# HighCWu/ControlLoRA

Measured on AMD Instinct MI355X. Metric: train images/sec SD-1.5+ControlLoRA 512^2 bs4/GPU, higher is better.
Workload: dtype f16; 1 GPU; configs/fill50k.json on SD-1.5 topology (seeded random weights), 512x512, bs=4/GPU, fp16; hot path = hint encoder + UNet fwd/bwd + adapter AdamW; latents/text embeddings synthetic (VAE/CLIP outside the hot path); global_batch=4, parallelism=dp1, hipgraph=True, allreduce_bytes=24188160, rccl_ranks=1, comm=torch, comm_requested=auto

## Files before the change

### controllora_amd/capi.py

```python
from __future__ import annotations

import ctypes as C
import os
from typing import Optional

import torch

_HERE = os.path.dirname(os.path.abspath(__file__))
LIB_PATH = os.environ.get("CLORA_LIB_PATH") or os.path.join(_HERE, "_build", "libclora.so")

ABI_VERSION = 4
OK, ERR_ARG, ERR_LAUNCH, ERR_WORKSPACE = 0, -1, -2, -3
_ERR = {ERR_ARG: "bad argument", ERR_LAUNCH: "kernel launch failed", ERR_WORKSPACE: "workspace too small"}


class CloraError(RuntimeError):
    pass


class ConvDesc(C.Structure):
    _fields_ = [(n, C.c_int) for n in (
        "enabled", "Hin", "Win", "Cin", "Hout", "Wout", "ksize", "mul", "kmul", "off", "lim_h", "lim_w", "shift",
        "need_even", "kchunk")]

# ... 90 lines not shown
    _fields_ = [("A", C.c_void_p), ("lda", C.c_int), ("T", C.c_void_p), ("ldt", C.c_int), ("toff", C.c_int), ("G", C.c_void_p),
                ("gs_n", C.c_int), ("gs_j", C.c_int), ("M", C.c_int), ("N", C.c_int), ("R", C.c_int), ("scale", C.c_float),
                ("a_rows", C.c_int), ("A2", C.c_void_p), ("lda2", C.c_int)]


class ConvPackJob(C.Structure):
    _fields_ = [("w", C.c_void_p), ("fwd", C.c_void_p), ("dgrad", C.c_void_p), ("Co", C.c_int), ("Ci", C.c_int), ("ksize", C.c_int),
                ("Cip", C.c_int), ("Cop", C.c_int), ("pad_", C.c_int)]


class ConvUnpackJob(C.Structure):
    _fields_ = [("stage", C.c_void_p), ("stage_b", C.c_void_p), ("grad_w", C.c_void_p), ("grad_b", C.c_void_p), ("Co", C.c_int),
                ("Ci", C.c_int), ("ksize", C.c_int), ("Cip", C.c_int)]


class SamplerCoef(C.Structure):
    _fields_ = [(n, C.c_float) for n in ("guidance", "x0_x", "x0_e", "k_x", "k_x0", "k_h", "k_e", "k_n")]


class ConvActJob(C.Structure):
    _fields_ = [("x", C.c_void_p), ("ldx", C.c_int), ("w", C.c_void_p), ("bias", C.c_void_p), ("y", C.c_void_p), ("ldy", C.c_int),
                ("Cin", C.c_int), ("Cout", C.c_int), ("relu", C.c_int)]


CONV_ACT_MAX_JOBS = 2
LORA_MAX_JOBS = 16
LORA_WGRAD_MAX_JOBS = 32
WGRAD_JOBS_PER_LAUNCH = min(LORA_WGRAD_MAX_JOBS, max(1, int(os.environ.get("CLORA_WGRAD_JOBS", "32"))))
CONV_MAX_JOBS = 32
CANNY_MAX_GROUP = 64
_P, _I, _Z, _F, _LL = C.c_void_p, C.c_int, C.c_size_t, C.c_float, C.c_longlong
_PROTOS = {
    "clora_gemm_f16": [_P, _I, _P, _P, _I, _I, _I, _I, C.POINTER(ConvDesc), C.POINTER(Epilogue), _I, _P, _Z, _P],
    "clora_gemm_f16_ex": [_P, _I, _P, _P, _I, _I, _I, _I, C.POINTER(ConvDesc), C.POINTER(Epilogue), _I, _I, _P, _Z, _P],
    "clora_conv_patch_eligible": [_I, C.POINTER(ConvDesc), _I],
    "clora_conv_strip_eligible": [_I, _I, C.POINTER(ConvDesc)],
    "clora_set_option": [C.c_char_p, _I],
    "clora_conv_wgrad_f16": [_P, _I, _P, _I, _P, _P, _I, _I, _I, C.POINTER(ConvDesc), _I, _P],
    "clora_conv_weight_pack_f32": [_P, _I, _I, _I, _I, _I, _P, _P, _P],
    "clora_conv_wgrad_unpack_f32": [_P, _P, _P, _P, _I, _I, _I, _I, _P],
    "clora_conv_weight_pack_multi_f32": [C.POINTER(ConvPackJob), _I, _P],
    "clora_conv_wgrad_unpack_multi_f32": [C.POINTER(ConvUnpackJob), _I, _P],
    "clora_attn_fwd_f16": [_P, _I, _P, _I, _P, _I, _P, _I, _P, _I, _I, _I, _I, _I, _F, _P],
    "clora_attn_max_head_dim": [_I],
    "clora_attn_fwd_causal_f16": [_P, _I, _P, _I, _P, _I, _P, _I, _I, _I, _I, _I, _F, _P],
    "clora_attn_bwd_f16": [_P, _I, _P, _I, _P, _I, _P, _I, _P, _I, _P, _P, _P, _I, _P, _I, _P, _I, _I, _I, _I, _I, _I, _F, _P, _Z, _P],
    "clora_groupnorm_fwd_f16": [_P, _P, _P, _P, _P, _I, _I, _I, _I, _F, _I, _P, _Z, _P],
    "clora_groupnorm_bwd_f16": [_P, _P, _P, _P, _P, _P, _P, _P, _P, _I, _I, _I, _I, _I, _I, _P, _Z, _P],
    "clora_groupnorm_fwd_f16_ex": [_P, _P, _I, C.POINTER(Deferred), _P, _P, _P, _P, _P, _I, _I, _I, _I, _F, _I, _P, _Z, _P],
    "clora_groupnorm_bwd_f16_ex": [_P, _P, C.POINTER(Deferred), _P, _P, _P, _I, _P, _P, _P, _P, _P, _I, _I, _I, _I, _I, _I, _P, _Z, _P],
    "clora_groupnorm_fwd_f16_team": [_P, _P, _I, C.POINTER(Deferred), _P, _P, _P, _P, _P, _I, _I, _I, _I, _F, _I, _P, _Z, _P, _Z, _P],
    "clora_groupnorm_fwd_f16_lo": [_P, _P, _I, C.POINTER(Deferred), _P, _P, _P, _P, _P, _I, _I, _I, _I, _F, _I, _P, _Z, _P, _Z, _P, _P, _P],
    "clora_layernorm_fwd_f16_lo": [_P, _P, _P, _P, _I, _I, _F, _P, _P],
    "clora_groupnorm_bwd_f16_team": [_P, _P, C.POINTER(Deferred), _P, _P, _P, _I, _P, _P, _P, _P, _P, _I, _I, _I, _I, _I, _I, _P, _Z, _P, _Z, _P],
    "clora_layernorm_bwd_f16_ex": [_P, _P, C.POINTER(Deferred), _P, _P, _P, _I, _I, _F, _P],
    "clora_finish_deferred": [C.POINTER(Deferred), _P],
    "clora_gemm_ln_fusable": [_I, _I, _I, _I, _I],
    "clora_gemm_tile_info": [_I, C.POINTER(GemmTile)],
    "clora_gemm_tile_at": [_I, C.POINTER(GemmTile)],
    "clora_gemm_fused_down_tile": [_I, _I, _I, C.POINTER(_I)],
    "clora_layernorm_fwd_f16": [_P, _P, _P, _P, _I, _I, _F, _P],
    "clora_softmax_rows_f16": [_P, _P, _I, _I, _I, _F, _P],
    "clora_layernorm_bwd_f16": [_P, _P, _P, _P, _P, _I, _I, _F, _P],
    "clora_geglu_fwd_f16": [_P, _P, _I, _I, _P],
    "clora_geglu_bwd_f16": [_P, _P, _P, _I, _I, _P],
    "clora_lora_down_f16": [_P, _I, _P, _I, _P, _I, _I, _I, _I, _I, _I, _I, _I, _F, _P],
    "clora_lora_down_multi_f16": [C.POINTER(LoraDownJob), _I, _P],
    "clora_lora_wgrad_multi_f16": [C.POINTER(LoraWgradJob), _I, _P, _Z, _P],
    "clora_lora_pack_f16": [_P, _I, _I, _P],
# ... 58 lines not shown
        self.cdll = C.CDLL(path)
        got = self.cdll.clora_abi_version() if hasattr(self.cdll, "clora_abi_version") else -1
        if got != ABI_VERSION and os.environ.get("CLORA_ABI_ANY", "") != "1":
            raise CloraError(f"{path} reports ABI {got}, this binding is written for ABI {ABI_VERSION} (include/clora.h); rebuild with "
                             "`python -m controllora_amd.build` (CLORA_ABI_ANY=1 overrides for A/B runs of older builds whose "
                             "struct layouts are known to match)")
        for name, argtypes in _PROTOS.items():
            if not hasattr(self.cdll, name) and os.environ.get("CLORA_ABI_ANY", "") == "1":
                continue
            fn = getattr(self.cdll, name)
            fn.argtypes = argtypes
            fn.restype = C.c_int
        self.cdll.clora_build_info.restype = C.c_char_p
        self.cdll.clora_groupnorm_workspace_bytes.restype = C.c_size_t
        self.cdll.clora_groupnorm_team_state_bytes.restype = C.c_size_t
        self.cdll.clora_lora_wgrad_workspace_bytes.restype = C.c_size_t
        self.cdll.clora_rank_gram_ws_bytes.restype = C.c_size_t
        if hasattr(self.cdll, "clora_conv_act_workspace"):
            self.cdll.clora_conv_act_workspace.restype = C.c_size_t
        self._options_from_env()
        self._derived = {}

    def derived(self, key, make):
        if key not in self._derived:
            self._derived[key] = make(self)
        return self._derived[key]

    def tiles(self) -> dict:
        def read(L):
            rows, r = {}, GemmTile()
# ... 58 lines not shown
```

### controllora_amd/csrc/clora_norm.hip

```cpp
#include <stdlib.h>
#include "clora_common.h"
#include "../../include/clora.h"
#include "clora_epilogue.h"

namespace {

constexpr int kMaxCols = 2;
constexpr int kLnCols = 4;

struct GnArgs {
    const half_t* x;
    const half_t* dy;
    const half_t* dres;
    half_t* y;
    const float* gamma;
    const float* beta;
    float* stats;
    float* partial;
    float* chpart;
    float* dgamma;
    float* dbeta;
    int B, HW, C, G, nchunk, rows_per_chunk;
    int accumulate_params;
    int params_in_apply;
// ... 464 lines not shown
                }
                if (r < r_end && cc < CH) {
                    const GnColW dc = gn_dx_col(p, cb + cc * 8);
                    st8(dc.p + ((size_t)b * p.HW + r) * dc.pitch, o);
                }
            }
        }
    }
}

__global__ __launch_bounds__(256) void gn_bwd_params_kernel(GnArgs p) {
    __shared__ float red[256 * 2];
    gn_bwd_params_block(p, blockIdx.x, red);
}

template <int NT>
__device__ __forceinline__ void gn_res_reduce(float* red, float* chs, const float (&a)[8], const float (&b)[8], int t, int CS, int cpg, int gps,
                                              int rl, int nrl, int c0, bool active, const float* weight, float* out2, float inv_n) {
    const int W = CS * 2;
    if (active) {
#pragma unroll
        for (int e = 0; e < 8; ++e) { red[rl * W + (c0 * 8 + e) * 2] = a[e]; red[rl * W + (c0 * 8 + e) * 2 + 1] = b[e]; }
    }
    __syncthreads();
    int seg = 1;
    while (seg < 8 && seg * 2 * CS <= NT) seg *= 2;
    {
        const int c = t / seg, sg = t - c * seg;
        float sa = 0.f, sb = 0.f;
        if (c < CS)
// ... 87 lines not shown
    gn_unpack8(ba, bb, bet);
    gn_affine8(mr, c0 * 8, cpg, gam, bet, sc, sh);
    half_t* ybase = p.y + (size_t)b * p.HW * p.C + cb + c0 * 8;
#pragma unroll
    for (int k = 0; k < NPT; ++k) {
        const int r = rl + k * nrl;
        half8 o;
        GN_NORM8(LO, v[k], w[k], lcol.m, sc, sh, p.fuse_silu, o)
        if (k < npt && r < p.HW) {
            st8(ybase + (size_t)r * p.C, o);
            if (p.xcopy) st8(p.xcopy + (size_t)b * p.HW * p.C + cb + c0 * 8 + (size_t)r * p.C, v[k]);
        }
    }
}

template <int NT, int NPT, bool DEF = false>
__global__ __launch_bounds__(NT) void gn_bwd_resident_kernel(GnArgs p) {
    __shared__ float red[NT * 16];
    __shared__ float chs[256 * 8 * 2];
    __shared__ float gs[64 * 2];
    const int t = threadIdx.x, b = blockIdx.z, cb = blockIdx.y * p.CS;
    const int CH = p.CS / 8, cpg = p.C / p.G, gps = p.G / p.nslab;
    const int nrl = NT / CH, rl = t / CH, c0 = t - rl * CH;
    const bool active = rl < nrl;
    const int npt = (p.HW + nrl - 1) / nrl;
    const size_t boff = (size_t)b * p.HW * p.C + cb + c0 * 8;
    float mean[8], rstd[8], sc[8], sh[8];
#pragma unroll
    for (int e = 0; e < 8; ++e) {
        const int ch = cb + (active ? c0 : 0) * 8 + e;
        const float* st = p.stats + ((size_t)b * p.G + ch / cpg) * 2;
// ... 21 lines not shown
#pragma unroll
        for (int k = 0; k < NPT; ++k) {
            const bool ok = k < npt && rl + k * nrl < p.HW;
#pragma unroll
            for (int e = 0; e < 8; ++e) {
                const float xf = (float)xv[k][e];
                const float xh = (xf - mean[e]) * rstd[e];
                float d = ok ? (float)gv[k][e] : 0.f;
                if (p.fuse_silu) d *= dsilu_f(xf * sc[e] + sh[e]);
                a1[e] += d;
                a2[e] += d * xh;
            }
        }
    }
    gn_res_reduce<NT>(red, chs, a1, a2, t, p.CS, cpg, gps, rl, nrl, c0, active, p.gamma + cb, gs, 1.0f / ((float)p.HW * (float)cpg));
    if (!active) return;
    float k2[8], k3[8];
#pragma unroll
    for (int e = 0; e < 8; ++e) {
        const int g = (c0 * 8 + e) / cpg;
        k2[e] = -rstd[e] * rstd[e] * gs[g * 2 + 1];
        k3[e] = -k2[e] * mean[e] - rstd[e] * gs[g * 2];
    }
    const bool has_res = p.dres != nullptr;
    const GnColW dxc = gn_dx_col(p, cb + c0 * 8);
#pragma unroll
    for (int k = 0; k < NPT; ++k) {
        const int r = rl + k * nrl;
        if (!(k < npt && r < p.HW)) continue;
        const size_t off = boff + (size_t)r * p.C;
// ... 119 lines not shown
    gn_unpack8(ba, bb, bet);
    gn_affine8(mr, c0 * 8, cpg, gam, bet, sc, sh);
    half_t* ybase = p.y + (size_t)b * p.HW * p.C + cb + c0 * 8;
#pragma unroll
    for (int k = 0; k < NPT; ++k) {
        const int r = r0 + rl + k * nrl;
        half8 o;
        GN_NORM8(LO, v[k], w[k], lcol.m, sc, sh, p.fuse_silu, o)
        if (r < r_end) {
            st8(ybase + (size_t)r * p.C, o);
            if (p.xcopy) st8(p.xcopy + (size_t)b * p.HW * p.C + cb + c0 * 8 + (size_t)r * p.C, v[k]);
        }
    }
}

template <int NT, int NPT>
__global__ __launch_bounds__(NT) void gn_bwd_team_kernel(GnArgs p) {
    __shared__ float red[NT * 16];
    __shared__ float chs[NT * 2];
    __shared__ float gs[64 * 2];
    __shared__ float gat[NT];
    __shared__ unsigned s_epoch;
    const int t = threadIdx.x;
    const int U = p.B * p.nslab, u = blockIdx.x % U, m = blockIdx.x / U;
    const int b = u / p.nslab, cb = (u - b * p.nslab) * p.CS;
    if (t == 0) s_epoch = CLORA_LD_AGENT_U32(p.tm_gen + u) + 1u;
    const int CH = p.CS / 8, cpg = p.C / p.G, gps = p.G / p.nslab;
    const int nrl = NT / CH, rl = t / CH, c0 = t - rl * CH;
    const bool active = rl < nrl;
    const int r0 = m * p.tm_rpb;
    const int r_end = (r0 + p.tm_rpb < p.HW) ? r0 + p.tm_rpb : p.HW;
// ... 22 lines not shown
#pragma unroll
        for (int k = 0; k < NPT; ++k) {
            const bool ok = r0 + rl + k * nrl < r_end;
#pragma unroll
            for (int e = 0; e < 8; ++e) {
                const float xf = (float)xv[k][e];
                const float xh = (xf - mean[e]) * rstd[e];
                float d = ok ? (float)gv[k][e] : 0.f;
                if (p.fuse_silu) d *= dsilu_f(xf * sc[e] + sh[e]);
                a1[e] += d;
                a2[e] += d * xh;
            }
        }
    }
    gn_res_reduce<NT>(red, chs, a1, a2, t, p.CS, cpg, gps, rl, nrl, c0, active, p.gamma + cb, gs, 1.0f);
    if (!gn_team_exchange<NT>(p, u, m, s_epoch, gps * 2, gs, gat, 1.0f / ((float)p.HW * (float)cpg))) return;
    if (!active) return;
    float k2[8], k3[8];
#pragma unroll
    for (int e = 0; e < 8; ++e) {
        const int g = (c0 * 8 + e) / cpg;
        k2[e] = -rstd[e] * rstd[e] * gs[g * 2 + 1];
        k3[e] = -k2[e] * mean[e] - rstd[e] * gs[g * 2];
    }
    const bool has_res = p.dres != nullptr;
    const GnColW dxc = gn_dx_col(p, cb + c0 * 8);
#pragma unroll
    for (int k = 0; k < NPT; ++k) {
        const int r = r0 + rl + k * nrl;
        if (!(r < r_end)) continue;
// ... 330 lines not shown
    }
}
size_t gn_workspace_bytes(const GnArgs& a, bool params) {
    size_t need = (size_t)a.B * a.nchunk * a.G * 2;
    if (params) need += (size_t)a.B * a.nchunk * a.C * 2;
    return need * sizeof(float);
}
int gn_bind_workspace(GnArgs& a, void* ws, size_t ws_bytes, bool params) {
    if (!ws || ws_bytes < gn_workspace_bytes(a, params)) return CLORA_ERR_WORKSPACE;
    a.partial = (float*)ws;
    a.chpart = params ? a.partial + (size_t)a.B * a.nchunk * a.G * 2 : nullptr;
    return CLORA_OK;
}

struct GnResident { int nt, npt; };
GnResident gn_resident_plan(GnArgs& a, bool bwd, bool params) {
    GnResident none = {0, 0};
    if (!clora_option(CLORA_OPT_GN_RESIDENT) || params) return none;
    const int cpg = a.C / a.G;
    int unit = 1;
    while ((unit * cpg) & 7) ++unit;
    if (a.G % unit) return none;
    int groups = unit;
    while (groups * cpg < 40 && groups * 2 <= a.G && a.G % (groups * 2) == 0) groups *= 2;
    const int CS = groups * cpg, CH = CS / 8;
    if (groups > 64 || CH > 256) return none;
    const int max_npt = bwd ? 8 : 16;
    for (int nt = 256; nt <= 512; nt *= 2) {
        const int nrl = nt / CH, npt = (a.HW + nrl - 1) / nrl;
        if (npt <= max_npt && groups * 8 <= nt && CS <= nt) {
            a.nslab = a.G / groups; a.CS = CS; a.nchunk = 1; a.rows_per_chunk = a.HW;
            GnResident r = {nt, npt <= 4 ? 4 : (npt <= 8 ? 8 : 16)};
            return r;
        }
    }
    return none;
}

int gn_team_plan(GnArgs& a, bool bwd, bool params, void* state, size_t state_bytes) {
    const int level = clora_option(CLORA_OPT_GN_TEAM);
    const int min_hw = level >= 4 ? 64 : ((level == 3 || (bwd && level == 2)) ? 256 : 1024);
    if (!state || state_bytes < kTeamStateBytes || params || !level || a.HW < min_hw) return 0;
    static int cus = -1;
    if (cus < 0) {
        int dev = 0, n = 0;
        if (hipGetDevice(&dev) != hipSuccess || hipDeviceGetAttribute(&n, hipDeviceAttributeMultiprocessorCount, dev) != hipSuccess) n = 0;
        cus = n;
    }
    if (cus < kTeamBlocks) return 0;
    const int cpg = a.C / a.G;
    int unit = 1;
    while ((unit * cpg) & 7) ++unit;
    if (a.G % unit) return 0;
    const int nunits = a.G / unit;
    int pick = 0, pick_npt = 0;
    for (int d = 1; d <= nunits; ++d) {
        if (nunits % d) continue;
        const int U = a.B * d;
        if (U > kTeamUnits || (kTeamBlocks % U)) continue;
        const int NB = kTeamBlocks / U, CS = a.C / d, CH = CS / 8, gps = a.G / d, GK = 2 * gps;
        if (NB < 2 || CS > kTeamNT || GK > kTeamGran || gps * 8 > kTeamNT) continue;
        if (NB > 8 * (kTeamNT / GK)) continue;
        const int nrl = kTeamNT / CH, rpb = clora_cdiv(a.HW, NB), npt = clora_cdiv(rpb, nrl);
        if (npt > (bwd ? 8 : 16)) continue;
        if (!pick || CS >= 160) { pick = d; pick_npt = npt; }
        if (CS < 160) break;
    }
    if (!pick) return 0;
    a.nslab = pick; a.CS = a.C / pick; a.nchunk = 1; a.rows_per_chunk = a.HW;
    a.tm_nb = kTeamBlocks / (a.B * pick); a.tm_rpb = clora_cdiv(a.HW, a.tm_nb);
    a.tm_err = (unsigned*)state; a.tm_gen = (unsigned*)((char*)state + 256);
    a.tm_gran = (unsigned long long*)((char*)state + kTeamHeader);
    a.tm_spin = 1u << 16; a.tm_probe = 0;
    return pick_npt <= 4 ? 4 : (pick_npt <= 8 ? 8 : 16);
}

enum GnForm { kGnTwoLaunch, kGnResident, kGnTeam };
struct GnLaunchPlan {
    GnForm form;
    int nt, npt;
    int nj, uf;
    bool deferred_here;
};
GnLaunchPlan gn_launch_plan(GnArgs& a, bool bwd, bool params, bool deferred, void* team_state, size_t team_state_bytes) {
    GnLaunchPlan pl = {kGnTwoLaunch, 0, 0, 1, 1, false};
    const GnResident res = gn_resident_plan(a, bwd, params);
    const bool fold_shape = res.nt && res.npt <= clora_option(CLORA_OPT_DEFER_MAX_ROWS);
    pl.deferred_here = deferred && fold_shape;
    if (!fold_shape && (!res.nt || clora_option(CLORA_OPT_GN_TEAM) >= 2)) {
        GnArgs ta = a;
        const int npt = gn_team_plan(ta, bwd, params, team_state, team_state_bytes);
        if (npt) {
            a = ta;
            pl.form = kGnTeam; pl.nt = kTeamNT; pl.npt = npt;
            return pl;
        }
    }
    if (res.nt) {
        pl.form = kGnResident; pl.nt = res.nt; pl.npt = res.npt;
        return pl;
    }
    gn_plan(a);
    pl.nj = a.CS / 8 > 256 ? 2 : 1;
    pl.uf = (pl.nj == 1 && clora_option(CLORA_OPT_GN_UNROLL)) ? 2 : 1;
    return pl;
}

template <bool BWD, bool DEF, bool LO>
void gn_resident_launch(const GnArgs& a, int nt, int npt, hipStream_t s) {
    static_assert(!(BWD && LO) && !(DEF && LO), "no such instantiation");
    const dim3 grid(1, a.nslab, a.B);
    if constexpr (BWD) {
        if (nt == 256 && npt == 4) hipLaunchKernelGGL((gn_bwd_resident_kernel<256, 4, DEF>), grid, dim3(256), 0, s, a);
        else if (nt == 256) hipLaunchKernelGGL((gn_bwd_resident_kernel<256, 8, DEF>), grid, dim3(256), 0, s, a);
        else hipLaunchKernelGGL((gn_bwd_resident_kernel<512, 8, DEF>), grid, dim3(512), 0, s, a);
    } else {
        if (nt == 256 && npt == 4) hipLaunchKernelGGL((gn_fwd_resident_kernel<256, 4, DEF, LO>), grid, dim3(256), 0, s, a);
        else if (nt == 256 && npt == 8) hipLaunchKernelGGL((gn_fwd_resident_kernel<256, 8, DEF, LO>), grid, dim3(256), 0, s, a);
        else if (nt == 256) hipLaunchKernelGGL((gn_fwd_resident_kernel<256, 16, DEF, LO>), grid, dim3(256), 0, s, a);
        else if (npt <= 8) hipLaunchKernelGGL((gn_fwd_resident_kernel<512, 8, DEF, LO>), grid, dim3(512), 0, s, a);
        else hipLaunchKernelGGL((gn_fwd_resident_kernel<512, 16, DEF, LO>), grid, dim3(512), 0, s, a);
    }
}

template <bool BWD, bool LO, int NJ, int UF>
void gn_two_launch_as(GnArgs& a, hipStream_t s) {
    const dim3 grid(a.nchunk, a.nslab, a.B), block(256);
    if constexpr (BWD) {
        static_assert(!LO, "no such instantiation");
        hipLaunchKernelGGL((gn_bwd_partial_kernel<NJ, UF>), grid, block, 0, s, a);
        a.params_in_apply = (a.dgamma && (long)a.nchunk * a.nslab * a.B >= clora_cdiv(a.C, 32)) ? 1 : 0;
        if (a.dgamma && !a.params_in_apply) hipLaunchKernelGGL(gn_bwd_params_kernel, dim3(clora_cdiv(a.C, 32)), block, 0, s, a);
        hipLaunchKernelGGL((gn_bwd_apply2_kernel<NJ, UF>), grid, block, 0, s, a);
    } else {
        hipLaunchKernelGGL((gn_fwd_partial_kernel<NJ, UF, LO>), grid, block, 0, s, a);
        hipLaunchKernelGGL((gn_fwd_apply2_kernel<NJ, UF, LO>), grid, block, 0, s, a);
    }
}
template <bool BWD, bool LO>
void gn_two_launch(GnArgs& a, int nj, int uf, hipStream_t s) {
    if (nj == 2) gn_two_launch_as<BWD, LO, 2, 1>(a, s);
    else if (uf == 2) gn_two_launch_as<BWD, LO, 1, 2>(a, s);
    else gn_two_launch_as<BWD, LO, 1, 1>(a, s);
}

template <bool BWD, bool LO = false>
void gn_team_launch(GnArgs& a, int npt, hipStream_t s) {
    const dim3 grid(kTeamBlocks), block(kTeamNT);
    for (int pass = CLORA_SEQUENTIAL_BLOCKS ? 0 : 1; pass < 2; ++pass) {
        a.tm_probe = pass == 0;
        if (BWD) {
            if (npt == 4) hipLaunchKernelGGL((gn_bwd_team_kernel<kTeamNT, 4>), grid, block, 0, s, a);
            else hipLaunchKernelGGL((gn_bwd_team_kernel<kTeamNT, 8>), grid, block, 0, s, a);
        } else {
            if (npt == 4) hipLaunchKernelGGL((gn_fwd_team_kernel<kTeamNT, 4, LO>), grid, block, 0, s, a);
            else if (npt == 8) hipLaunchKernelGGL((gn_fwd_team_kernel<kTeamNT, 8, LO>), grid, block, 0, s, a);
            else hipLaunchKernelGGL((gn_fwd_team_kernel<kTeamNT, 16, LO>), grid, block, 0, s, a);
        }
    }
}

int ew_blocks(size_t n) {
    size_t b = (n + 255) / 256;
    return (int)(b > 4096 ? 4096 : (b < 1 ? 1 : b));
}

}

// ... 22 lines not shown
    const bool lo = x_lo || x2_lo;
    if (lo && src && src->splits > 0) return CLORA_ERR_ARG;
    if (!gn_shape_ok(B, HW, C, G)) return CLORA_ERR_ARG;
    hipStream_t s = (hipStream_t)stream;
    const bool deferred = src && src->splits > 0;
    if (deferred) {
        if (x2 || !deferred_fits(src, B * HW, C)) return CLORA_ERR_ARG;
        x = src->C;
    }
    if (!x || (x2 && (Ca <= 0 || Ca >= C || (Ca & 7)))) return CLORA_ERR_ARG;
    GnArgs a = GnArgs();
    a.x = (const half_t*)x; a.y = (half_t*)y; a.gamma = gamma; a.beta = beta; a.stats = stats;
    a.B = B; a.HW = HW; a.C = C; a.G = G; a.eps = eps; a.fuse_silu = fuse_silu;
    a.x2 = (const half_t*)x2; a.Ca = x2 ? Ca : C; a.xcopy = (half_t*)xcopy;
    a.x_lo = (const half_t*)x_lo; a.x2_lo = (const half_t*)x2_lo;
    const GnLaunchPlan pl = gn_launch_plan(a, false, false, deferred, team_state, team_state_bytes);
    if (deferred && !pl.deferred_here) {
        const int rc = clora_finish_deferred(src, stream);
        if (rc != CLORA_OK) return rc;
    }
    if (pl.form == kGnTeam) {
        if (lo) gn_team_launch<false, true>(a, pl.npt, s);
        else gn_team_launch<false>(a, pl.npt, s);
    } else if (pl.form == kGnResident) {
        if (pl.deferred_here) {
            a.fin_partial = src->partial; a.fin_splits = src->splits; a.fin_epi = src->epi; a.xcopy = (half_t*)src->C;
            gn_resident_launch<false, true, false>(a, pl.nt, pl.npt, s);
        } else if (lo) {
            gn_resident_launch<false, false, true>(a, pl.nt, pl.npt, s);
        } else {
            gn_resident_launch<false, false, false>(a, pl.nt, pl.npt, s);
// ... 31 lines not shown
    return gn_fwd_impl(x, x2, Ca, src, xcopy, y, gamma, beta, stats, B, HW, C, G, eps, fuse_silu, team_state, team_state_bytes, workspace,
                       workspace_bytes, stream, x_lo, x2_lo);
}

extern "C" int clora_groupnorm_fwd_f16(const clora_half* x, clora_half* y, const float* gamma, const float* beta,
                                       float* stats, int B, int HW, int C, int G, float eps, int fuse_silu,
                                       void* workspace, size_t workspace_bytes, void* stream) {
    return clora_groupnorm_fwd_f16_ex(x, nullptr, 0, nullptr, nullptr, y, gamma, beta, stats, B, HW, C, G, eps, fuse_silu, workspace,
                                      workspace_bytes, stream);
}

namespace {
int gn_bwd_impl(const clora_half* x, const clora_half* dy, const clora_deferred_t* dy_src, const clora_half* dres,
                clora_half* dx, clora_half* dx2, int Ca, const float* gamma, const float* beta,
                const float* stats, float* dgamma, float* dbeta, int B, int HW, int C, int G, int fuse_silu,
                int accumulate_params, void* team_state, size_t team_state_bytes, void* workspace, size_t workspace_bytes, void* stream) {
    if (!x || !dx || !gamma || !beta || !stats || ((dgamma == nullptr) != (dbeta == nullptr))) return CLORA_ERR_ARG;
    if (!gn_shape_ok(B, HW, C, G)) return CLORA_ERR_ARG;
    if (dx2 && (Ca <= 0 || Ca >= C || (Ca & 7))) return CLORA_ERR_ARG;
    const bool deferred = dy_src && dy_src->splits > 0;
    if (deferred) {
        if (!deferred_fits(dy_src, B * HW, C)) return CLORA_ERR_ARG;
        dy = dy_src->C;
    }
    if (!dy) return CLORA_ERR_ARG;
    GnArgs a = GnArgs();
    a.x = (const half_t*)x; a.dy = (const half_t*)dy; a.dres = (const half_t*)dres; a.y = (half_t*)dx; a.gamma = gamma; a.beta = beta;
    a.stats = const_cast<float*>(stats); a.dgamma = dgamma; a.dbeta = dbeta;
    a.B = B; a.HW = HW; a.C = C; a.G = G; a.fuse_silu = fuse_silu; a.accumulate_params = accumulate_params;
    a.y2 = (half_t*)dx2; a.Ca = dx2 ? Ca : C;
    hipStream_t s = (hipStream_t)stream;
    const bool params = dgamma != nullptr;
    const GnLaunchPlan pl = gn_launch_plan(a, true, params, deferred, team_state, team_state_bytes);
    if (deferred && !pl.deferred_here) {
        const int rc = clora_finish_deferred(dy_src, stream);
        if (rc != CLORA_OK) return rc;
    }
    if (pl.form == kGnTeam) {
        gn_team_launch<true>(a, pl.npt, s);
    } else if (pl.form == kGnResident) {
        if (pl.deferred_here) {
            a.fin_partial = dy_src->partial; a.fin_splits = dy_src->splits; a.fin_epi = dy_src->epi;
            gn_resident_launch<true, true, false>(a, pl.nt, pl.npt, s);
        } else {
            gn_resident_launch<true, false, false>(a, pl.nt, pl.npt, s);
        }
    } else {
        const int rc = gn_bind_workspace(a, workspace, workspace_bytes, params);
        if (rc != CLORA_OK) return rc;
        gn_two_launch<true, false>(a, pl.nj, pl.uf, s);
    }
    return clora_check_launch();
}
}

extern "C" int clora_groupnorm_bwd_f16_ex(const clora_half* x, const clora_half* dy, const clora_deferred_t* dy_src, const clora_half* dres,
                                          clora_half* dx, clora_half* dx2, int Ca, const float* gamma, const float* beta,
                                          const float* stats, float* dgamma, float* dbeta, int B, int HW, int C, int G, int fuse_silu,
                                          int accumulate_params, void* workspace, size_t workspace_bytes, void* stream) {
    return gn_bwd_impl(x, dy, dy_src, dres, dx, dx2, Ca, gamma, beta, stats, dgamma, dbeta, B, HW, C, G, fuse_silu, accumulate_params, nullptr, 0,
                       workspace, workspace_bytes, stream);
}

extern "C" int clora_groupnorm_bwd_f16_team(const clora_half* x, const clora_half* dy, const clora_deferred_t* dy_src, const clora_half* dres,
                                            clora_half* dx, clora_half* dx2, int Ca, const float* gamma, const float* beta,
                                            const float* stats, float* dgamma, float* dbeta, int B, int HW, int C, int G, int fuse_silu,
                                            int accumulate_params, void* team_state, size_t team_state_bytes, void* workspace,
                                            size_t workspace_bytes, void* stream) {
    return gn_bwd_impl(x, dy, dy_src, dres, dx, dx2, Ca, gamma, beta, stats, dgamma, dbeta, B, HW, C, G, fuse_silu, accumulate_params, team_state,
                       team_state_bytes, workspace, workspace_bytes, stream);
}

extern "C" int clora_groupnorm_bwd_f16(const clora_half* x, const clora_half* dy, const clora_half* dres, clora_half* dx, const float* gamma,
                                       const float* beta, const float* stats, float* dgamma, float* dbeta, int B,
                                       int HW, int C, int G, int fuse_silu, int accumulate_params, void* workspace,
                                       size_t workspace_bytes, void* stream) {
    return clora_groupnorm_bwd_f16_ex(x, dy, nullptr, dres, dx, nullptr, 0, gamma, beta, stats, dgamma, dbeta, B, HW, C, G, fuse_silu,
                                      accumulate_params, workspace, workspace_bytes, stream);
}

namespace {
int ln_fwd_impl(const clora_half* x, clora_half* y, const float* gamma, const float* beta, int M, int C, float eps,
                const clora_half* x_lo, void* stream) {
    if (!x || !y || !gamma || !beta || M <= 0 || C <= 0 || (C & 7) || C / 8 > 64 * kLnCols) return CLORA_ERR_ARG;
    LnArgs a = LnArgs();
// ... 55 lines not shown
```

### controllora_amd/kernels.py

```python
from __future__ import annotations

import ctypes as C
import os
from typing import Optional, Tuple

import torch

from . import capi
from .capi import ConvDesc, Epilogue, ptr

f16, f32 = torch.float16, torch.float32


class KernelProfiler:

    def __init__(self, detail=False):
        self.detail = detail
        self.records = []

    def summary(self):
        torch.cuda.synchronize()
        agg = {}
        for name, e0, e1, fl, by in self.records:
            a = agg.setdefault(name, dict(calls=0, ms=0.0, flops=0.0, bytes=0.0))
# ... 482 lines not shown
    if split_at:
        dx = torch.empty((B, HW, split_at), dtype=f16, device=x.device)
        dx2 = torch.empty((B, HW, Cc - split_at), dtype=f16, device=x.device)
    else:
        dx, dx2 = torch.empty_like(x), None
    dg = db = None
    if grads_into is not None:
        dg, db = grads_into
        want_param_grads = True
    elif want_param_grads:
        dg = torch.empty(Cc, dtype=f32, device=x.device)
        db = torch.empty(Cc, dtype=f32, device=x.device)
    ws = _gn_ws(B, HW, Cc, G, x.device, True, want_param_grads)
    assert dres is None or (dres.shape == x.shape and dres.is_contiguous())
    team = gn_team_state(x.device)
    _call("clora_groupnorm_bwd_f16_team", ptr(x, f16), ptr(dy, f16), C.byref(dy_src) if dy_src is not None else None,
          ptr(dres, f16) if dres is not None else None, ptr(dx), ptr(dx2) if dx2 is not None else None, int(split_at),
          ptr(gamma, f32), ptr(beta, f32), ptr(stats, f32),
          ptr(dg, f32) if dg is not None else None, ptr(db, f32) if db is not None else None, B, HW, Cc, G, int(silu),
          int(grads_into is not None), ptr(team), team.numel(), ptr(ws), ws.numel())
    if split_at:
        dx = (dx, dx2)
    return (dx, None, None) if grads_into is not None else (dx, dg, db)


def layernorm_fwd(x, gamma, beta, eps, x_lo=None):
    x2 = _c2(x)
    y = torch.empty_like(x)
    if x_lo is not None:
        assert x_lo.shape == x.shape and x_lo.is_contiguous()
        _call("clora_layernorm_fwd_f16_lo", ptr(x2, f16), ptr(y), ptr(gamma, f32), ptr(beta, f32), x2.shape[0], x2.shape[1], float(eps),
              ptr(x_lo, f16))
        return y
    _call("clora_layernorm_fwd_f16", ptr(x2, f16), ptr(y), ptr(gamma, f32), ptr(beta, f32), x2.shape[0], x2.shape[1], float(eps))
    return y


def layernorm_bwd(x, dy, gamma, eps, dres=None):
# ... 183 lines not shown


def lora_wgrad_multi(jobs, device):
    groups = {}
    for j in jobs:
        groups.setdefault(4 if j.R <= 4 else (8 if j.R <= 8 else 16), []).append(j)
    wsb = capi.lib().cdll.clora_lora_wgrad_workspace_bytes
    for _, js in groups.items():
        for i in range(0, len(js), capi.WGRAD_JOBS_PER_LAUNCH):
            chunk = js[i:i + capi.WGRAD_JOBS_PER_LAUNCH]
            ws = workspace(sum(wsb(j.M, j.N, j.R) for j in chunk), device)
            arr = (capi.LoraWgradJob * len(chunk))(*chunk)
            _call("clora_lora_wgrad_multi_f16", arr, len(chunk), ptr(ws), ws.numel(), nbytes=sum(2.0 * j.M * j.N for j in chunk))


_wgrad_queue = {"jobs": [], "refs": [], "task": None, "enabled": os.environ.get("CLORA_DEFER_WGRAD", "1") != "0", "unpack": []}
DEFER_UNPACK = os.environ.get("CLORA_DEFER_UNPACK", "1") != "0"


def _graph_task_id():
    f = getattr(torch._C, "_current_graph_task_id", None)
    return f() if f is not None else -1


def _defer_open():
    if not _wgrad_queue["enabled"] or PROFILER is not None:
        return False
    task = _graph_task_id()
    if task < 0:
        return False
    if _wgrad_queue["task"] != task:
        lora_wgrad_discard()
# ... 10 lines not shown
    _wgrad_queue["refs"].extend(keepalive)
    _wgrad_queue["device"] = device


def conv_unpack_defer(job, *keepalive) -> bool:
    if not DEFER_UNPACK or not _defer_open():
        return False
    _wgrad_queue["unpack"].append(job)
    _wgrad_queue["refs"].extend(keepalive)
    return True


def lora_wgrad_discard():
    _wgrad_queue["jobs"].clear()
    _wgrad_queue["unpack"].clear()
    _wgrad_queue["refs"].clear()
    _wgrad_queue["task"] = None


def lora_wgrad_flush():
    jobs, _wgrad_queue["jobs"] = _wgrad_queue["jobs"], []
    unpack, _wgrad_queue["unpack"] = _wgrad_queue["unpack"], []
    _wgrad_queue["task"] = None
    if unpack:
        conv_wgrad_unpack_multi(unpack)
    if jobs:
        batches = []
        for j in jobs:
            for b in batches:
                if len(b[0]) < capi.WGRAD_JOBS_PER_LAUNCH and j.G not in b[1] and b[2] == (4 if j.R <= 4 else (8 if j.R <= 8 else 16)):
                    b[0].append(j); b[1].add(j.G)
                    break
            else:
                batches.append(([j], {j.G}, 4 if j.R <= 4 else (8 if j.R <= 8 else 16)))
        for b in batches:
            lora_wgrad_multi(b[0], _wgrad_queue["device"])
    _wgrad_queue["refs"].clear()


def lora_up(base, T, toff, U, M, N, scale, out=None, u_tr=False):
# ... 267 lines not shown
```

### include/clora.h

```cpp
#ifndef CLORA_H
#define CLORA_H
#include <stddef.h>
#include <stdint.h>

#ifdef __cplusplus
extern "C" {
#endif

#define CLORA_OK 0
#define CLORA_ERR_ARG (-1)
#define CLORA_ERR_LAUNCH (-2)
#define CLORA_ERR_WORKSPACE (-3)

typedef uint16_t clora_half;

typedef struct {
    int enabled;
    int Hin, Win, Cin;
    int Hout, Wout;
    int ksize;
    int mul, kmul, off, lim_h, lim_w, shift, need_even;
    int kchunk;
} clora_conv_t;

// ... 136 lines not shown
int clora_groupnorm_bwd_f16_ex(const clora_half* x, const clora_half* dy, const clora_deferred_t* dy_src, const clora_half* dres,
                               clora_half* dx, clora_half* dx2, int Ca, const float* gamma, const float* beta, const float* stats,
                               float* dgamma, float* dbeta, int B, int HW, int C, int G, int fuse_silu, int accumulate_params,
                               void* workspace, size_t workspace_bytes, void* stream);

size_t clora_groupnorm_team_state_bytes(void);
int clora_groupnorm_fwd_f16_team(const clora_half* x, const clora_half* x2, int Ca, const clora_deferred_t* src, clora_half* xcopy,
                                 clora_half* y, const float* gamma, const float* beta, float* stats, int B, int HW, int C, int G,
                                 float eps, int fuse_silu, void* team_state, size_t team_state_bytes, void* workspace,
                                 size_t workspace_bytes, void* stream);
int clora_groupnorm_bwd_f16_team(const clora_half* x, const clora_half* dy, const clora_deferred_t* dy_src, const clora_half* dres,
                                 clora_half* dx, clora_half* dx2, int Ca, const float* gamma, const float* beta, const float* stats,
                                 float* dgamma, float* dbeta, int B, int HW, int C, int G, int fuse_silu, int accumulate_params,
                                 void* team_state, size_t team_state_bytes, void* workspace, size_t workspace_bytes, void* stream);

int clora_groupnorm_fwd_f16_lo(const clora_half* x, const clora_half* x2, int Ca, const clora_deferred_t* src, clora_half* xcopy,
                               clora_half* y, const float* gamma, const float* beta, float* stats, int B, int HW, int C, int G,
                               float eps, int fuse_silu, void* team_state, size_t team_state_bytes, void* workspace,
                               size_t workspace_bytes, const clora_half* x_lo, const clora_half* x2_lo, void* stream);
int clora_layernorm_fwd_f16_lo(const clora_half* x, clora_half* y, const float* gamma, const float* beta, int M, int C,
                               float eps, const clora_half* x_lo, void* stream);

int clora_softmax_rows_f16(const clora_half* x, clora_half* y, int rows, int cols, int ld, float scale, void* stream);

int clora_layernorm_fwd_f16(const clora_half* x, clora_half* y, const float* gamma, const float* beta, int M, int C,
                            float eps, void* stream);
int clora_layernorm_bwd_f16(const clora_half* x, const clora_half* dy, const clora_half* dres, clora_half* dx,
                            const float* gamma, int M, int C, float eps, void* stream);
int clora_layernorm_bwd_f16_ex(const clora_half* x, const clora_half* dy, const clora_deferred_t* dy_src, const clora_half* dres,
                               clora_half* dx, const float* gamma, int M, int C, float eps, void* stream);
// ... 164 lines not shown
```

Before: 181.3 images/s.

## Let GroupNorm backward with param grads use resident/team kernels via slot partials and batched fold

GroupNorm backward that needs dgamma/dbeta was previously barred from the resident and team single-pass kernels and fell back to the two-launch path. Those kernels now write per-batch (or per-team-block) channel partials into a slots buffer. A new multi-job fold kernel reduces the partials into dgamma/dbeta, and when accumulating, folds are deferred and batched with the queued wgrad flush. The cost is an extra slots allocation per call plus a fold launch, and the fold introduces more deferred-state bookkeeping.

```diff
diff --git a/controllora_amd/capi.py b/controllora_amd/capi.py
--- a/controllora_amd/capi.py
+++ b/controllora_amd/capi.py
@@ -128,6 +128,11 @@
                 ("Ci", C.c_int), ("ksize", C.c_int), ("Cip", C.c_int)]
 
 
+class GnFoldJob(C.Structure):
+    _fields_ = [("chpart", C.c_void_p * 4), ("nslots", C.c_int * 4), ("dgamma", C.c_void_p), ("dbeta", C.c_void_p), ("C", C.c_int),
+                ("nregions", C.c_int), ("accumulate", C.c_int), ("pad_", C.c_int)]
+
+
 class SamplerCoef(C.Structure):
     _fields_ = [(n, C.c_float) for n in ("guidance", "x0_x", "x0_e", "k_x", "k_x0", "k_h", "k_e", "k_n")]
 
@@ -142,6 +147,8 @@
 LORA_WGRAD_MAX_JOBS = 32
 WGRAD_JOBS_PER_LAUNCH = min(LORA_WGRAD_MAX_JOBS, max(1, int(os.environ.get("CLORA_WGRAD_JOBS", "32"))))
 CONV_MAX_JOBS = 32
+GN_FOLD_MAX_JOBS = 32
+GN_FOLD_MAX_REGIONS = 4
 CANNY_MAX_GROUP = 64
 _P, _I, _Z, _F, _LL = C.c_void_p, C.c_int, C.c_size_t, C.c_float, C.c_longlong
 _PROTOS = {
@@ -167,6 +174,10 @@
     "clora_groupnorm_fwd_f16_lo": [_P, _P, _I, C.POINTER(Deferred), _P, _P, _P, _P, _P, _I, _I, _I, _I, _F, _I, _P, _Z, _P, _Z, _P, _P, _P],
     "clora_layernorm_fwd_f16_lo": [_P, _P, _P, _P, _I, _I, _F, _P, _P],
     "clora_groupnorm_bwd_f16_team": [_P, _P, C.POINTER(Deferred), _P, _P, _P, _I, _P, _P, _P, _P, _P, _I, _I, _I, _I, _I, _I, _P, _Z, _P, _Z, _P],
+    "clora_groupnorm_bwd_f16_slots": [_P, _P, C.POINTER(Deferred), _P, _P, _P, _I, _P, _P, _P, _P, _P, _I, _I, _I, _I, _I, _I, _P, _Z, _P, _Z,
+                                      _P, _Z, C.POINTER(_I), _P],
+    "clora_groupnorm_param_fold_multi_f32": [C.POINTER(GnFoldJob), _I, _P],
+    "clora_groupnorm_param_slots_bytes": [_I, _I],
     "clora_layernorm_bwd_f16_ex": [_P, _P, C.POINTER(Deferred), _P, _P, _P, _I, _I, _F, _P],
     "clora_finish_deferred": [C.POINTER(Deferred), _P],
     "clora_gemm_ln_fusable": [_I, _I, _I, _I, _I],
@@ -255,6 +266,8 @@
         self.cdll.clora_build_info.restype = C.c_char_p
         self.cdll.clora_groupnorm_workspace_bytes.restype = C.c_size_t
         self.cdll.clora_groupnorm_team_state_bytes.restype = C.c_size_t
+        if hasattr(self.cdll, "clora_groupnorm_param_slots_bytes"):
+            self.cdll.clora_groupnorm_param_slots_bytes.restype = C.c_size_t
         self.cdll.clora_lora_wgrad_workspace_bytes.restype = C.c_size_t
         self.cdll.clora_rank_gram_ws_bytes.restype = C.c_size_t
         if hasattr(self.cdll, "clora_conv_act_workspace"):
diff --git a/controllora_amd/csrc/clora_norm.hip b/controllora_amd/csrc/clora_norm.hip
--- a/controllora_amd/csrc/clora_norm.hip
+++ b/controllora_amd/csrc/clora_norm.hip
@@ -502,6 +502,22 @@
     gn_bwd_params_block(p, blockIdx.x, red);
 }
 
+struct GnFoldJobs { clora_gn_fold_job_t j[CLORA_GN_FOLD_MAX_JOBS]; };
+__global__ __launch_bounds__(256) void gn_param_fold_multi_kernel(GnFoldJobs jobs) {
+    __shared__ float red[256 * 2];
+    const clora_gn_fold_job_t& job = jobs.j[blockIdx.y];
+    if ((int)blockIdx.x * 32 >= job.C) return;
+    for (int r = 0; r < job.nregions; ++r) {
+        GnArgs q = GnArgs();
+        q.chpart = const_cast<float*>(job.chpart[r]);
+        q.B = 1; q.nchunk = job.nslots[r]; q.C = job.C;
+        q.dgamma = job.dgamma; q.dbeta = job.dbeta;
+        q.accumulate_params = (r > 0 || job.accumulate) ? 1 : 0;
+        if (r > 0) __syncthreads();
+        gn_bwd_params_block(q, blockIdx.x, red);
+    }
+}
+
 template <int NT>
 __device__ __forceinline__ void gn_res_reduce(float* red, float* chs, const float (&a)[8], const float (&b)[8], int t, int CS, int cpg, int gps,
                                               int rl, int nrl, int c0, bool active, const float* weight, float* out2, float inv_n) {
@@ -619,7 +635,7 @@
     }
 }
 
-template <int NT, int NPT, bool DEF = false>
+template <int NT, int NPT, bool DEF = false, bool PAR = false>
 __global__ __launch_bounds__(NT) void gn_bwd_resident_kernel(GnArgs p) {
     __shared__ float red[NT * 16];
     __shared__ float chs[256 * 8 * 2];
@@ -671,6 +687,10 @@
         }
     }
     gn_res_reduce<NT>(red, chs, a1, a2, t, p.CS, cpg, gps, rl, nrl, c0, active, p.gamma + cb, gs, 1.0f / ((float)p.HW * (float)cpg));
+    if constexpr (PAR) {
+        float* slot = p.chpart + ((size_t)b * p.C + cb) * 2;
+        for (int i = t; i < p.CS * 2; i += NT) slot[i] = chs[i];
+    }
     if (!active) return;
     float k2[8], k3[8];
 #pragma unroll
@@ -820,7 +840,7 @@
     }
 }
 
-template <int NT, int NPT>
+template <int NT, int NPT, bool PAR = false>
 __global__ __launch_bounds__(NT) void gn_bwd_team_kernel(GnArgs p) {
     __shared__ float red[NT * 16];
     __shared__ float chs[NT * 2];
@@ -873,6 +893,10 @@
         }
     }
     gn_res_reduce<NT>(red, chs, a1, a2, t, p.CS, cpg, gps, rl, nrl, c0, active, p.gamma + cb, gs, 1.0f);
+    if constexpr (PAR) {
+        float* slot = p.chpart + (((size_t)b * p.tm_nb + m) * p.C + cb) * 2;
+        for (int i = t; i < p.CS * 2; i += NT) slot[i] = chs[i];
+    }
     if (!gn_team_exchange<NT>(p, u, m, s_epoch, gps * 2, gs, gat, 1.0f / ((float)p.HW * (float)cpg))) return;
     if (!active) return;
     float k2[8], k3[8];
@@ -1233,9 +1257,9 @@
 }
 
 struct GnResident { int nt, npt; };
-GnResident gn_resident_plan(GnArgs& a, bool bwd, bool params) {
+GnResident gn_resident_plan(GnArgs& a, bool bwd, bool params, long slot_cap) {
     GnResident none = {0, 0};
-    if (!clora_option(CLORA_OPT_GN_RESIDENT) || params) return none;
+    if (!clora_option(CLORA_OPT_GN_RESIDENT) || (params && slot_cap < a.B)) return none;
     const int cpg = a.C / a.G;
     int unit = 1;
     while ((unit * cpg) & 7) ++unit;
@@ -1256,10 +1280,10 @@
     return none;
 }
 
-int gn_team_plan(GnArgs& a, bool bwd, bool params, void* state, size_t state_bytes) {
+int gn_team_plan(GnArgs& a, bool bwd, bool params, long slot_cap, void* state, size_t state_bytes) {
     const int level = clora_option(CLORA_OPT_GN_TEAM);
     const int min_hw = level >= 4 ? 64 : ((level == 3 || (bwd && level == 2)) ? 256 : 1024);
-    if (!state || state_bytes < kTeamStateBytes || params || !level || a.HW < min_hw) return 0;
+    if (!state || state_bytes < kTeamStateBytes || !level || a.HW < min_hw) return 0;
     static int cus = -1;
     if (cus < 0) {
         int dev = 0, n = 0;
@@ -1282,6 +1306,7 @@
         if (NB > 8 * (kTeamNT / GK)) continue;
         const int nrl = kTeamNT / CH, rpb = clora_cdiv(a.HW, NB), npt = clora_cdiv(rpb, nrl);
         if (npt > (bwd ? 8 : 16)) continue;
+        if (params && slot_cap < (long)a.B * NB) continue;
         if (!pick || CS >= 160) { pick = d; pick_npt = npt; }
         if (CS < 160) break;
     }
@@ -1301,14 +1326,14 @@
     int nj, uf;
     bool deferred_here;
 };
-GnLaunchPlan gn_launch_plan(GnArgs& a, bool bwd, bool params, bool deferred, void* team_state, size_t team_state_bytes) {
+GnLaunchPlan gn_launch_plan(GnArgs& a, bool bwd, bool params, long slot_cap, bool deferred, void* team_state, size_t team_state_bytes) {
     GnLaunchPlan pl = {kGnTwoLaunch, 0, 0, 1, 1, false};
-    const GnResident res = gn_resident_plan(a, bwd, params);
+    const GnResident res = gn_resident_plan(a, bwd, params, slot_cap);
     const bool fold_shape = res.nt && res.npt <= clora_option(CLORA_OPT_DEFER_MAX_ROWS);
     pl.deferred_here = deferred && fold_shape;
     if (!fold_shape && (!res.nt || clora_option(CLORA_OPT_GN_TEAM) >= 2)) {
         GnArgs ta = a;
-        const int npt = gn_team_plan(ta, bwd, params, team_state, team_state_bytes);
+        const int npt = gn_team_plan(ta, bwd, params, slot_cap, team_state, team_state_bytes);
         if (npt) {
             a = ta;
             pl.form = kGnTeam; pl.nt = kTeamNT; pl.npt = npt;
@@ -1325,14 +1350,14 @@
     return pl;
 }
 
-template <bool BWD, bool DEF, bool LO>
+template <bool BWD, bool DEF, bool LO, bool PAR = false>
 void gn_resident_launch(const GnArgs& a, int nt, int npt, hipStream_t s) {
-    static_assert(!(BWD && LO) && !(DEF && LO), "no such instantiation");
+    static_assert(!(BWD && LO) && !(DEF && LO) && !(PAR && !BWD), "no such instantiation");
     const dim3 grid(1, a.nslab, a.B);
     if constexpr (BWD) {
-        if (nt == 256 && npt == 4) hipLaunchKernelGGL((gn_bwd_resident_kernel<256, 4, DEF>), grid, dim3(256), 0, s, a);
-        else if (nt == 256) hipLaunchKernelGGL((gn_bwd_resident_kernel<256, 8, DEF>), grid, dim3(256), 0, s, a);
-        else hipLaunchKernelGGL((gn_bwd_resident_kernel<512, 8, DEF>), grid, dim3(512), 0, s, a);
+        if (nt == 256 && npt == 4) hipLaunchKernelGGL((gn_bwd_resident_kernel<256, 4, DEF, PAR>), grid, dim3(256), 0, s, a);
+        else if (nt == 256) hipLaunchKernelGGL((gn_bwd_resident_kernel<256, 8, DEF, PAR>), grid, dim3(256), 0, s, a);
+        else hipLaunchKernelGGL((gn_bwd_resident_kernel<512, 8, DEF, PAR>), grid, dim3(512), 0, s, a);
     } else {
         if (nt == 256 && npt == 4) hipLaunchKernelGGL((gn_fwd_resident_kernel<256, 4, DEF, LO>), grid, dim3(256), 0, s, a);
         else if (nt == 256 && npt == 8) hipLaunchKernelGGL((gn_fwd_resident_kernel<256, 8, DEF, LO>), grid, dim3(256), 0, s, a);
@@ -1363,14 +1388,14 @@
     else gn_two_launch_as<BWD, LO, 1, 1>(a, s);
 }
 
-template <bool BWD, bool LO = false>
+template <bool BWD, bool LO = false, bool PAR = false>
 void gn_team_launch(GnArgs& a, int npt, hipStream_t s) {
     const dim3 grid(kTeamBlocks), block(kTeamNT);
     for (int pass = CLORA_SEQUENTIAL_BLOCKS ? 0 : 1; pass < 2; ++pass) {
         a.tm_probe = pass == 0;
         if (BWD) {
-            if (npt == 4) hipLaunchKernelGGL((gn_bwd_team_kernel<kTeamNT, 4>), grid, block, 0, s, a);
-            else hipLaunchKernelGGL((gn_bwd_team_kernel<kTeamNT, 8>), grid, block, 0, s, a);
+            if (npt == 4) hipLaunchKernelGGL((gn_bwd_team_kernel<kTeamNT, 4, PAR>), grid, block, 0, s, a);
+            else hipLaunchKernelGGL((gn_bwd_team_kernel<kTeamNT, 8, PAR>), grid, block, 0, s, a);
         } else {
             if (npt == 4) hipLaunchKernelGGL((gn_fwd_team_kernel<kTeamNT, 4, LO>), grid, block, 0, s, a);
             else if (npt == 8) hipLaunchKernelGGL((gn_fwd_team_kernel<kTeamNT, 8, LO>), grid, block, 0, s, a);
@@ -1423,7 +1448,7 @@
     a.B = B; a.HW = HW; a.C = C; a.G = G; a.eps = eps; a.fuse_silu = fuse_silu;
     a.x2 = (const half_t*)x2; a.Ca = x2 ? Ca : C; a.xcopy = (half_t*)xcopy;
     a.x_lo = (const half_t*)x_lo; a.x2_lo = (const half_t*)x2_lo;
-    const GnLaunchPlan pl = gn_launch_plan(a, false, false, deferred, team_state, team_state_bytes);
+    const GnLaunchPlan pl = gn_launch_plan(a, false, false, 0, deferred, team_state, team_state_bytes);
     if (deferred && !pl.deferred_here) {
         const int rc = clora_finish_deferred(src, stream);
         if (rc != CLORA_OK) return rc;
@@ -1485,7 +1510,9 @@
 int gn_bwd_impl(const clora_half* x, const clora_half* dy, const clora_deferred_t* dy_src, const clora_half* dres,
                 clora_half* dx, clora_half* dx2, int Ca, const float* gamma, const float* beta,
                 const float* stats, float* dgamma, float* dbeta, int B, int HW, int C, int G, int fuse_silu,
-                int accumulate_params, void* team_state, size_t team_state_bytes, void* workspace, size_t workspace_bytes, void* stream) {
+                int accumulate_params, void* team_state, size_t team_state_bytes, void* workspace, size_t workspace_bytes, void* stream,
+                float* slots = nullptr, size_t slots_bytes = 0, int* nslots = nullptr) {
+    if (nslots) *nslots = 0;
     if (!x || !dx || !gamma || !beta || !stats || ((dgamma == nullptr) != (dbeta == nullptr))) return CLORA_ERR_ARG;
     if (!gn_shape_ok(B, HW, C, G)) return CLORA_ERR_ARG;
     if (dx2 && (Ca <= 0 || Ca >= C || (Ca & 7))) return CLORA_ERR_ARG;
@@ -1502,19 +1529,28 @@
     a.y2 = (half_t*)dx2; a.Ca = dx2 ? Ca : C;
     hipStream_t s = (hipStream_t)stream;
     const bool params = dgamma != nullptr;
-    const GnLaunchPlan pl = gn_launch_plan(a, true, params, deferred, team_state, team_state_bytes);
+    const long slot_cap = (params && slots && nslots) ? (long)(slots_bytes / ((size_t)C * 2 * sizeof(float))) : 0;
+    const GnLaunchPlan pl = gn_launch_plan(a, true, params, slot_cap, deferred, team_state, team_state_bytes);
     if (deferred && !pl.deferred_here) {
         const int rc = clora_finish_deferred(dy_src, stream);
         if (rc != CLORA_OK) return rc;
     }
     if (pl.form == kGnTeam) {
-        gn_team_launch<true>(a, pl.npt, s);
+        if (params) {
+            a.chpart = slots; *nslots = a.B * a.tm_nb;
+            gn_team_launch<true, false, true>(a, pl.npt, s);
+        } else {
+            gn_team_launch<true>(a, pl.npt, s);
+        }
     } else if (pl.form == kGnResident) {
+        if (params) { a.chpart = slots; *nslots = a.B; }
         if (pl.deferred_here) {
             a.fin_partial = dy_src->partial; a.fin_splits = dy_src->splits; a.fin_epi = dy_src->epi;
-            gn_resident_launch<true, true, false>(a, pl.nt, pl.npt, s);
+            if (params) gn_resident_launch<true, true, false, true>(a, pl.nt, pl.npt, s);
+            else gn_resident_launch<true, true, false>(a, pl.nt, pl.npt, s);
         } else {
-            gn_resident_launch<true, false, false>(a, pl.nt, pl.npt, s);
+            if (params) gn_resident_launch<true, false, false, true>(a, pl.nt, pl.npt, s);
+            else gn_resident_launch<true, false, false>(a, pl.nt, pl.npt, s);
         }
     } else {
         const int rc = gn_bind_workspace(a, workspace, workspace_bytes, params);
@@ -1540,6 +1576,39 @@
                                             size_t workspace_bytes, void* stream) {
     return gn_bwd_impl(x, dy, dy_src, dres, dx, dx2, Ca, gamma, beta, stats, dgamma, dbeta, B, HW, C, G, fuse_silu, accumulate_params, team_state,
                        team_state_bytes, workspace, workspace_bytes, stream);
+}
+
+extern "C" size_t clora_groupnorm_param_slots_bytes(int B, int C) {
+    if (B <= 0 || C <= 0) return 0;
+    return (size_t)(B > kTeamBlocks ? B : kTeamBlocks) * C * 2 * sizeof(float);
+}
+
+extern "C" int clora_groupnorm_bwd_f16_slots(const clora_half* x, const clora_half* dy, const clora_deferred_t* dy_src, const clora_half* dres,
+                                             clora_half* dx, clora_half* dx2, int Ca, const float* gamma, const float* beta,
+                                             const float* stats, float* dgamma, float* dbeta, int B, int HW, int C, int G, int fuse_silu,
+                                             int accumulate_params, void* team_state, size_t team_state_bytes, void* workspace,
+                                             size_t workspace_bytes, float* slots, size_t slots_bytes, int* nslots, void* stream) {
+    if (!dgamma || !dbeta || !slots || !nslots) return CLORA_ERR_ARG;
+    return gn_bwd_impl(x, dy, dy_src, dres, dx, dx2, Ca, gamma, beta, stats, dgamma, dbeta, B, HW, C, G, fuse_silu, accumulate_params, team_state,
+                       team_state_bytes, workspace, workspace_bytes, stream, slots, slots_bytes, nslots);
+}
+
+extern "C" int clora_groupnorm_param_fold_multi_f32(const clora_gn_fold_job_t* jobs, int njobs, void* stream) {
+    if (!jobs || njobs <= 0 || njobs > CLORA_GN_FOLD_MAX_JOBS) return CLORA_ERR_ARG;
+    GnFoldJobs fj;
+    int maxC = 0;
+    for (int i = 0; i < njobs; ++i) {
+        const clora_gn_fold_job_t& j = jobs[i];
+        if (!j.dgamma || !j.dbeta || j.C <= 0 || j.nregions <= 0 || j.nregions > CLORA_GN_FOLD_MAX_REGIONS) return CLORA_ERR_ARG;
+        for (int r = 0; r < j.nregions; ++r)
+            if (!j.chpart[r] || j.nslots[r] <= 0) return CLORA_ERR_ARG;
+        for (int k = 0; k < i; ++k)
+            if (jobs[k].dgamma == j.dgamma || jobs[k].dbeta == j.dbeta) return CLORA_ERR_ARG;
+        fj.j[i] = j;
+        if (j.C > maxC) maxC = j.C;
+    }
+    hipLaunchKernelGGL(gn_param_fold_multi_kernel, dim3(clora_cdiv(maxC, 32), njobs), dim3(256), 0, (hipStream_t)stream, fj);
+    return clora_check_launch();
 }
 
 extern "C" int clora_groupnorm_bwd_f16(const clora_half* x, const clora_half* dy, const clora_half* dres, clora_half* dx, const float* gamma,
diff --git a/controllora_amd/kernels.py b/controllora_amd/kernels.py
--- a/controllora_amd/kernels.py
+++ b/controllora_amd/kernels.py
@@ -520,14 +520,51 @@
     ws = _gn_ws(B, HW, Cc, G, x.device, True, want_param_grads)
     assert dres is None or (dres.shape == x.shape and dres.is_contiguous())
     team = gn_team_state(x.device)
-    _call("clora_groupnorm_bwd_f16_team", ptr(x, f16), ptr(dy, f16), C.byref(dy_src) if dy_src is not None else None,
-          ptr(dres, f16) if dres is not None else None, ptr(dx), ptr(dx2) if dx2 is not None else None, int(split_at),
-          ptr(gamma, f32), ptr(beta, f32), ptr(stats, f32),
-          ptr(dg, f32) if dg is not None else None, ptr(db, f32) if db is not None else None, B, HW, Cc, G, int(silu),
-          int(grads_into is not None), ptr(team), team.numel(), ptr(ws), ws.numel())
+    args = (ptr(x, f16), ptr(dy, f16), C.byref(dy_src) if dy_src is not None else None,
+            ptr(dres, f16) if dres is not None else None, ptr(dx), ptr(dx2) if dx2 is not None else None, int(split_at),
+            ptr(gamma, f32), ptr(beta, f32), ptr(stats, f32),
+            ptr(dg, f32) if dg is not None else None, ptr(db, f32) if db is not None else None, B, HW, Cc, G, int(silu),
+            int(grads_into is not None), ptr(team), team.numel(), ptr(ws), ws.numel())
+    if want_param_grads and GN_PARAM_SLOTS and hasattr(capi.lib().cdll, "clora_groupnorm_bwd_f16_slots"):
+        slots = torch.empty(capi.lib().cdll.clora_groupnorm_param_slots_bytes(B, Cc) // 4, dtype=f32, device=x.device)
+        nslots = C.c_int(0)
+        _call("clora_groupnorm_bwd_f16_slots", *args, ptr(slots), slots.numel() * 4, C.byref(nslots))
+        if nslots.value > 0:
+            gn_fold_defer(slots, nslots.value, dg, db, Cc, grads_into is not None)
+    else:
+        _call("clora_groupnorm_bwd_f16_team", *args)
     if split_at:
         dx = (dx, dx2)
     return (dx, None, None) if grads_into is not None else (dx, dg, db)
+
+
+GN_PARAM_SLOTS = os.environ.get("CLORA_GN_PARAM_SLOTS", "1") != "0"
+
+
+def gn_param_fold_multi(jobs):
+    while jobs:
+        now, later = jobs[:capi.GN_FOLD_MAX_JOBS], jobs[capi.GN_FOLD_MAX_JOBS:]
+        arr = (capi.GnFoldJob * len(now))()
+        for j, (dg, db, Cc, acc, regions) in zip(arr, now):
+            head, rest = regions[:capi.GN_FOLD_MAX_REGIONS], regions[capi.GN_FOLD_MAX_REGIONS:]
+            for r, (slots, n) in enumerate(head):
+                j.chpart[r], j.nslots[r] = ptr(slots, f32), n
+            j.dgamma, j.dbeta, j.C, j.nregions, j.accumulate = ptr(dg, f32), ptr(db, f32), Cc, len(head), int(acc)
+            if rest:
+                later.append((dg, db, Cc, True, rest))
+        _call("clora_groupnorm_param_fold_multi_f32", arr, len(now))
+        jobs = later
+
+
+def gn_fold_defer(slots, nslots, dg, db, Cc, accumulate):
+    if not (accumulate and DEFER_GN_FOLD and _defer_open()):
+        gn_param_fold_multi([(dg, db, Cc, accumulate, [(slots, nslots)])])
+        return
+    key = (dg.data_ptr(), db.data_ptr())
+    job = _wgrad_queue["gn_fold"].get(key)
+    if job is None:
+        job = _wgrad_queue["gn_fold"][key] = (dg, db, Cc, True, [])
+    job[4].append((slots, nslots))
 
 
 def layernorm_fwd(x, gamma, beta, eps, x_lo=None):
@@ -741,8 +778,9 @@
             _call("clora_lora_wgrad_multi_f16", arr, len(chunk), ptr(ws), ws.numel(), nbytes=sum(2.0 * j.M * j.N for j in chunk))
 
 
-_wgrad_queue = {"jobs": [], "refs": [], "task": None, "enabled": os.environ.get("CLORA_DEFER_WGRAD", "1") != "0", "unpack": []}
+_wgrad_queue = {"jobs": [], "refs": [], "task": None, "enabled": os.environ.get("CLORA_DEFER_WGRAD", "1") != "0", "unpack": [], "gn_fold": {}}
 DEFER_UNPACK = os.environ.get("CLORA_DEFER_UNPACK", "1") != "0"
+DEFER_GN_FOLD = os.environ.get("CLORA_DEFER_GN_FOLD", "1") != "0"
 
 
 def _graph_task_id():
@@ -783,6 +821,7 @@
 def lora_wgrad_discard():
     _wgrad_queue["jobs"].clear()
     _wgrad_queue["unpack"].clear()
+    _wgrad_queue["gn_fold"].clear()
     _wgrad_queue["refs"].clear()
     _wgrad_queue["task"] = None
 
@@ -790,9 +829,12 @@
 def lora_wgrad_flush():
     jobs, _wgrad_queue["jobs"] = _wgrad_queue["jobs"], []
     unpack, _wgrad_queue["unpack"] = _wgrad_queue["unpack"], []
+    gn_fold, _wgrad_queue["gn_fold"] = _wgrad_queue["gn_fold"], {}
     _wgrad_queue["task"] = None
     if unpack:
         conv_wgrad_unpack_multi(unpack)
+    if gn_fold:
+        gn_param_fold_multi(list(gn_fold.values()))
     if jobs:
         batches = []
         for j in jobs:
diff --git a/include/clora.h b/include/clora.h
--- a/include/clora.h
+++ b/include/clora.h
@@ -174,6 +174,23 @@
                                  float* dgamma, float* dbeta, int B, int HW, int C, int G, int fuse_silu, int accumulate_params,
                                  void* team_state, size_t team_state_bytes, void* workspace, size_t workspace_bytes, void* stream);
 
+#define CLORA_GN_FOLD_MAX_JOBS 32
+#define CLORA_GN_FOLD_MAX_REGIONS 4
+typedef struct {
+    const float* chpart[CLORA_GN_FOLD_MAX_REGIONS];
+    int nslots[CLORA_GN_FOLD_MAX_REGIONS];
+    float* dgamma;
+    float* dbeta;
+    int C, nregions, accumulate, pad_;
+} clora_gn_fold_job_t;
+size_t clora_groupnorm_param_slots_bytes(int B, int C);
+int clora_groupnorm_bwd_f16_slots(const clora_half* x, const clora_half* dy, const clora_deferred_t* dy_src, const clora_half* dres,
+                                  clora_half* dx, clora_half* dx2, int Ca, const float* gamma, const float* beta, const float* stats,
+                                  float* dgamma, float* dbeta, int B, int HW, int C, int G, int fuse_silu, int accumulate_params,
+                                  void* team_state, size_t team_state_bytes, void* workspace, size_t workspace_bytes, float* slots,
+                                  size_t slots_bytes, int* nslots, void* stream);
+int clora_groupnorm_param_fold_multi_f32(const clora_gn_fold_job_t* jobs, int njobs, void* stream);
+
 int clora_groupnorm_fwd_f16_lo(const clora_half* x, const clora_half* x2, int Ca, const clora_deferred_t* src, clora_half* xcopy,
                                clora_half* y, const float* gamma, const float* beta, float* stats, int B, int HW, int C, int G,
                                float eps, int fuse_silu, void* team_state, size_t team_state_bytes, void* workspace,
```

Result: no change. 181.8 images/s, median of 6 (+0.3%).
